# One-2-3-45/One-2-3-45

Measured on NVIDIA H100. Metric: sec/mesh end-to-end (256x256 in), lower is better.
Workload: dtype f16

## Files before the change

### one-2-3-45_b200/csrc/gemm_tc.cu

```cuda
#include <cuda.h>
#include <stdlib.h>
#include <cuda_fp16.h>

#include "common.cuh"
#include "wgmma.cuh"

namespace o2345 {
namespace {

constexpr int BM = 128, BK = 64;
constexpr int EPI_WARPS = 8;
constexpr int EPI_THREADS = 32 * EPI_WARPS;
constexpr int GEMM_THREADS = 128 + EPI_THREADS;
constexpr uint64_t WAIT_LIMIT_NS = 4000000000ull;
constexpr int MAX_CLUSTER = 8;
constexpr int RES_PREFETCH = 8;

enum { WAIT_EMPTY = 1, WAIT_FULL = 2 };

struct TrapRecord {
  unsigned long long magic;
  int tag, stage, bx, by, bz, rank, M, N, K, bn, mode, splits, conv;
};
constexpr unsigned long long TRAP_MAGIC = 0x6f32333435545250ull;
// ... 16 lines not shown
      "mbarrier.try_wait.parity.shared::cta.b64 p, [%1], %2;\n\t"
      "selp.u32 %0, 1, 0, p;\n\t}"
      : "=r"(done)
      : "r"(smem_u32(bar)), "r"(parity)
      : "memory");
  return done;
}
__device__ __forceinline__ uint64_t global_ns() {
  uint64_t t;
  asm volatile("mov.u64 %0, %%globaltimer;" : "=l"(t));
  return t;
}
__device__ __forceinline__ void tma_load_2d(void* dst, const CUtensorMap* map, uint64_t* bar, int c0, int c1) {
  asm volatile(
      "cp.async.bulk.tensor.2d.shared::cluster.global.mbarrier::complete_tx::bytes [%0], [%1, {%3, %4}], [%2];"
      ::"r"(smem_u32(dst)), "l"(map), "r"(smem_u32(bar)), "r"(c0), "r"(c1)
      : "memory");
}
__device__ __forceinline__ void tma_load_4d(void* dst, const CUtensorMap* map, uint64_t* bar, int c0, int c1, int c2, int c3) {
  asm volatile(
      "cp.async.bulk.tensor.4d.shared::cluster.global.mbarrier::complete_tx::bytes [%0], [%1, {%3, %4, %5, %6}], [%2];"
      ::"r"(smem_u32(dst)), "l"(map), "r"(smem_u32(bar)), "r"(c0), "r"(c1), "r"(c2), "r"(c3)
      : "memory");
}
__device__ __forceinline__ uint32_t cluster_ctarank() {
  uint32_t r;
  asm volatile("mov.u32 %0, %%cluster_ctarank;" : "=r"(r));
  return r;
}
__device__ __forceinline__ void cluster_sync_all() {
  asm volatile("barrier.cluster.arrive.release.aligned;\n\tbarrier.cluster.wait.acquire.aligned;" ::: "memory");
}
__device__ __forceinline__ void epi_bar() { asm volatile("bar.sync 1, 256;" ::: "memory"); }

__host__ __device__ constexpr int acc_ld(int bn) { return bn + 4; }
__device__ __forceinline__ void acc_ld32(const float* src, uint32_t (&r)[32]) {
#pragma unroll
  for (int i = 0; i < 8; ++i) {
    const float4 v = reinterpret_cast<const float4*>(src)[i];
    r[4 * i] = __float_as_uint(v.x), r[4 * i + 1] = __float_as_uint(v.y), r[4 * i + 2] = __float_as_uint(v.z), r[4 * i + 3] = __float_as_uint(v.w);
  }
}

struct GemmParams {
  int M, N, K;
  int64_t ldc;
  int nh;
  int64_t stride_c_h, stride_c_b;
  const float* bias;
  const __half* rowbias;
  int64_t rowbias_ld;
  int rows_per_group;
  const __half* residual;
  void* C;
  int out_f32;
  int act;
  float alpha;
  int batched;
  int conv, cC, cH, cW, cblocks;
  int ctaps, ctx, cox, coy, up, upa, upb;
  int splits;
  float* ws;
  int persist;
  long long* trace;
  TrapRecord* diag;
  int bn, mode;
};

__device__ __forceinline__ void stamp(const GemmParams& p, int slot) {
  if (p.trace && blockIdx.x == 0 && blockIdx.y == 0 && blockIdx.z == 0) p.trace[slot] = clock64();
}
__device__ __forceinline__ void stamp_ns(const GemmParams& p, int slot, bool any_z = false) {
  if (p.trace && blockIdx.x == 0 && blockIdx.y == 0 && (any_z || blockIdx.z == 0)) p.trace[slot] = (long long)global_ns();
}

__device__ __forceinline__ int64_t out_row(const GemmParams& p, int row) {
  if (!p.up) return row;
  const int x = row % p.cW, t = row / p.cW, y = t % p.cH, b = t / p.cH;
  return ((int64_t)b * (2 * p.cH) + 2 * y + p.upa) * (2 * p.cW) + 2 * x + p.upb;
}

__device__ __noinline__ void wait_timed_out(const GemmParams& p, int tag, int stage) {
  if (p.diag) {
    TrapRecord* d = p.diag;
    d->tag = tag, d->stage = stage, d->bx = blockIdx.x, d->by = blockIdx.y, d->bz = blockIdx.z, d->rank = (int)cluster_ctarank();
    d->M = p.M, d->N = p.N, d->K = p.K, d->bn = p.bn, d->mode = p.mode, d->splits = p.splits, d->conv = p.conv;
    __threadfence_system();
    d->magic = TRAP_MAGIC;
    __threadfence_system();
  }
  __trap();
}
__device__ __forceinline__ void mbar_wait(uint64_t* bar, uint32_t parity, const GemmParams& p, int tag, int stage) {
  if (mbar_try(bar, parity)) return;
  const uint64_t t0 = global_ns();
  uint32_t spins = 0;
  while (!mbar_try(bar, parity))
    if (((++spins) & 255u) == 0 && global_ns() - t0 > WAIT_LIMIT_NS) wait_timed_out(p, tag, stage);
}

__device__ __forceinline__ float gelu_erf(float x) { return 0.5f * x * (1.f + erff(x * 0.70710678118654752f)); }
__device__ __forceinline__ float gelu_erf_fast(float x) {
  const float z = fabsf(x) * 0.70710678118654752f;
  const float t = __fdividef(1.f, fmaf(0.3275911f, z, 1.f));
  const float poly = t * fmaf(t, fmaf(t, fmaf(t, fmaf(t, 1.061405429f, -1.453152027f), 1.421413741f), -0.284496736f), 0.254829592f);
  float e;
  asm("ex2.approx.ftz.f32 %0, %1;" : "=f"(e) : "f"(-z * z * 1.4426950408889634f));
  const float erf_abs = fmaf(-poly, e, 1.f);
  return 0.5f * x * (1.f + copysignf(erf_abs, x));
}
__device__ __forceinline__ float apply_act(float x, int act) {
  if (act == 1) return x / (1.f + __expf(-x));
  if (act == 2) return gelu_erf(x);
  if (act == 4) return x / (1.f + __expf(-1.702f * x));
  return x;
}

__device__ __forceinline__ void store8(const GemmParams& p, int64_t off, const float (&v)[8]) {
  if (p.out_f32) {
    float* o = reinterpret_cast<float*>(p.C) + off;
    *reinterpret_cast<float4*>(o) = make_float4(v[0], v[1], v[2], v[3]);
    *reinterpret_cast<float4*>(o + 4) = make_float4(v[4], v[5], v[6], v[7]);
  } else {
    __half2 h[4];
#pragma unroll
    for (int e = 0; e < 4; ++e) h[e] = __floats2half2_rn(v[2 * e], v[2 * e + 1]);
    *reinterpret_cast<uint4*>(reinterpret_cast<__half*>(p.C) + off) = *reinterpret_cast<uint4*>(h);
  }
}

__device__ __forceinline__ void epilogue_chunk(const GemmParams& p, const uint32_t (&r)[32], int row, int64_t crow, int col0) {
  const __half* rb = p.rowbias ? p.rowbias + (int64_t)(row / p.rows_per_group) * p.rowbias_ld : nullptr;
  if (p.act == 3) {
    if (col0 >= p.N) return;
    float v[16];
#pragma unroll
    for (int e = 0; e < 16; ++e) {
      float a = __uint_as_float(r[e]) * p.alpha, g = __uint_as_float(r[16 + e]) * p.alpha;
      if (p.bias) a += __ldg(p.bias + col0 + e), g += __ldg(p.bias + col0 + 16 + e);
      v[e] = a * gelu_erf(g);
    }
    const int64_t o = crow + (col0 >> 1);
    float lo[8], hi[8];
#pragma unroll
    for (int e = 0; e < 8; ++e) lo[e] = v[e], hi[e] = v[8 + e];
    store8(p, o, lo);
    store8(p, o + 8, hi);
    return;
  }
#pragma unroll
  for (int j = 0; j < 32; j += 8) {
    const int col = col0 + j;
    if (col >= p.N) break;
    float v[8];
    const bool full = col + 8 <= p.N;
    if (full && rb) {
      uint4 q = *reinterpret_cast<const uint4*>(rb + col);
      const __half* h = reinterpret_cast<const __half*>(&q);
#pragma unroll
      for (int e = 0; e < 8; ++e) v[e] = __half2float(h[e]);
    } else {
#pragma unroll
      for (int e = 0; e < 8; ++e) v[e] = (rb && col + e < p.N) ? __half2float(rb[col + e]) : 0.f;
    }
#pragma unroll
    for (int e = 0; e < 8; ++e) {
      float x = fmaf(__uint_as_float(r[j + e]), p.alpha, v[e]);
      if (p.bias && col + e < p.N) x += __ldg(p.bias + col + e);
      v[e] = apply_act(x, p.act);
    }
    if (full && (p.ldc & 7) == 0) {
      if (p.residual) {
        uint4 q = *reinterpret_cast<const uint4*>(p.residual + crow + col);
        const __half* h = reinterpret_cast<const __half*>(&q);
#pragma unroll
        for (int e = 0; e < 8; ++e) v[e] += __half2float(h[e]);
      }
      store8(p, crow + col, v);
    } else {
      for (int e = 0; e < 8 && col + e < p.N; ++e) {
        float x = v[e];
        if (p.residual) x += __half2float(p.residual[crow + col + e]);
        if (p.out_f32) reinterpret_cast<float*>(p.C)[crow + col + e] = x;
        else reinterpret_cast<__half*>(p.C)[crow + col + e] = __float2half_rn(x);
      }
    }
  }
}

__device__ __forceinline__ void splitk_partial(const GemmParams& p, const uint32_t (&r)[32], int split, int row, int col0) {
  float* w = p.ws + ((int64_t)split * p.M + row) * p.N + col0;
  if ((p.N & 3) == 0) {
#pragma unroll
    for (int e = 0; e < 32; e += 4)
      if (col0 + e < p.N)
        __stcg(reinterpret_cast<float4*>(w + e), make_float4(__uint_as_float(r[e]), __uint_as_float(r[e + 1]),
                                                              __uint_as_float(r[e + 2]), __uint_as_float(r[e + 3])));
  } else {
#pragma unroll
    for (int e = 0; e < 32; ++e)
      if (col0 + e < p.N) __stcg(w + e, __uint_as_float(r[e]));
  }
}

template <int BN>
__device__ __forceinline__ void splitk_finalize(const GemmParams& p, int m0, int n0, int z, int te) {
  const bool vec = (p.N % 8) == 0 && (p.ldc % 8) == 0 && (!p.rowbias || (p.rowbias_ld % 8) == 0);
  const int64_t plane = (int64_t)p.M * p.N;
  if (vec) {
    constexpr int PPR = BN / 8;
    constexpr int NP = BM * PPR;
    const int share = (NP + p.splits - 1) / p.splits;
    const int i1 = min(NP, (z + 1) * share);
    constexpr bool FIXED_COLS = (EPI_THREADS % PPR) == 0;
    float bcol[8];
#pragma unroll
    for (int e = 0; e < 8; ++e) bcol[e] = 0.f;
    if (FIXED_COLS && p.bias) {
      const int i0 = z * share + te, col = n0 + (i0 - (i0 / PPR) * PPR) * 8;
      if (col < p.N) {
        const float4 b0 = __ldg(reinterpret_cast<const float4*>(p.bias + col)), b1 = __ldg(reinterpret_cast<const float4*>(p.bias + col + 4));
        bcol[0] = b0.x, bcol[1] = b0.y, bcol[2] = b0.z, bcol[3] = b0.w, bcol[4] = b1.x, bcol[5] = b1.y, bcol[6] = b1.z, bcol[7] = b1.w;
      }
    }
    for (int i = z * share + te; i < i1; i += EPI_THREADS) {
      const int rl = i / PPR, row = m0 + rl, col = n0 + (i - rl * PPR) * 8;
      if (row >= p.M || col >= p.N) continue;
      const int64_t woff = (int64_t)row * p.N + col, o = out_row(p, row) * p.ldc + col;
      uint4 qb = make_uint4(0u, 0u, 0u, 0u), qr = make_uint4(0u, 0u, 0u, 0u);
      if (p.rowbias) qb = *reinterpret_cast<const uint4*>(p.rowbias + (int64_t)(row / p.rows_per_group) * p.rowbias_ld + col);
      if (p.residual) qr = *reinterpret_cast<const uint4*>(p.residual + o);
      if (!FIXED_COLS && p.bias) {
        const float4 b0 = __ldg(reinterpret_cast<const float4*>(p.bias + col)), b1 = __ldg(reinterpret_cast<const float4*>(p.bias + col + 4));
        bcol[0] = b0.x, bcol[1] = b0.y, bcol[2] = b0.z, bcol[3] = b0.w, bcol[4] = b1.x, bcol[5] = b1.y, bcol[6] = b1.z, bcol[7] = b1.w;
// ... 23 lines not shown
        v[e] = apply_act(x, p.act);
      }
      if (p.residual) {
        const __half* h = reinterpret_cast<const __half*>(&qr);
#pragma unroll
        for (int e = 0; e < 8; ++e) v[e] += __half2float(h[e]);
      }
      store8(p, o, v);
    }
    return;
  }
  const int share = (BM * BN + p.splits - 1) / p.splits;
  const int i1 = min(BM * BN, (z + 1) * share);
  for (int i = z * share + te; i < i1; i += EPI_THREADS) {
    const int rl = i / BN, row = m0 + rl, col = n0 + (i - rl * BN);
    if (row >= p.M || col >= p.N) continue;
    float x = 0.f;
    for (int s = 0; s < p.splits; ++s) x += __ldcg(p.ws + (int64_t)s * plane + (int64_t)row * p.N + col);
    x *= p.alpha;
    if (p.rowbias) x += __half2float(p.rowbias[(int64_t)(row / p.rows_per_group) * p.rowbias_ld + col]);
    if (p.bias) x += __ldg(p.bias + col);
    x = apply_act(x, p.act);
    const int64_t o = out_row(p, row) * p.ldc + col;
    if (p.residual) x += __half2float(p.residual[o]);
    if (p.out_f32) reinterpret_cast<float*>(p.C)[o] = x;
    else reinterpret_cast<__half*>(p.C)[o] = __float2half_rn(x);
  }
}

constexpr int EPI_RB_GROUPS = 8;
__host__ __device__ constexpr int epi_smem_bytes(int bn) { return bn * 4 + EPI_RB_GROUPS * bn * 2; }
__host__ __device__ constexpr int col_split(int bn) { return ((bn / 2 + 31) / 32) * 32; }

template <int BN>
__device__ __forceinline__ void epilogue_preload(const GemmParams& p, int m0, int n0, float* sbias, __half* srb, int te) {
  for (int i = te; i < BN; i += EPI_THREADS) sbias[i] = (p.bias && n0 + i < p.N) ? __ldg(p.bias + n0 + i) : 0.f;
  if (p.rowbias) {
    const int g0 = m0 / p.rows_per_group;
    const int last = (m0 + BM - 1 < p.M ? m0 + BM - 1 : p.M - 1) / p.rows_per_group;
    const int ng = last - g0 + 1;
    if (ng >= 1 && ng <= EPI_RB_GROUPS)
      for (int i = te; i < ng * BN; i += EPI_THREADS) {
        const int gi = i / BN, c = i - gi * BN;
        srb[i] = (n0 + c < p.N) ? p.rowbias[(int64_t)(g0 + gi) * p.rowbias_ld + n0 + c] : __float2half(0.f);
      }
  }
  epi_bar();
}

template <int ACT>
__device__ __forceinline__ float act_fn(float x) {
  if (ACT == 1) return __fdividef(x, 1.f + __expf(-x));
  if (ACT == 2) return gelu_erf(x);
  if (ACT == 4) return __fdividef(x, 1.f + __expf(-1.702f * x));
  return x;
}

template <int ACT>
__device__ __forceinline__ void stage_rows(const GemmParams& p, const float* acc_row, uint8_t* mine, int n0, int c_lo, int c_hi,
                                           const float* sbias, const __half* rb, bool rb_smem) {
#pragma unroll 1
  for (int c0 = c_lo; c0 < c_hi; c0 += 32) {
    if (n0 + c0 >= p.N) break;
    uint32_t r[32];
    acc_ld32(acc_row + c0, r);
    if (ACT == 3) {
      __half2 h[8];
#pragma unroll
      for (int e = 0; e < 16; e += 2) {
        float a0 = fmaf(__uint_as_float(r[e]), p.alpha, sbias[c0 + e]), a1 = fmaf(__uint_as_float(r[e + 1]), p.alpha, sbias[c0 + e + 1]);
        float g0 = fmaf(__uint_as_float(r[16 + e]), p.alpha, sbias[c0 + 16 + e]);
        float g1 = fmaf(__uint_as_float(r[17 + e]), p.alpha, sbias[c0 + 17 + e]);
        h[e >> 1] = __floats2half2_rn(a0 * gelu_erf_fast(g0), a1 * gelu_erf_fast(g1));
      }
      uint4* d = reinterpret_cast<uint4*>(mine + (c0 - c_lo));
      d[0] = reinterpret_cast<uint4*>(h)[0], d[1] = reinterpret_cast<uint4*>(h)[1];
    } else {
#pragma unroll
      for (int j = 0; j < 32; j += 8) {
        float v[8];
        const float4 b0 = *reinterpret_cast<const float4*>(sbias + c0 + j), b1 = *reinterpret_cast<const float4*>(sbias + c0 + j + 4);
        v[0] = b0.x, v[1] = b0.y, v[2] = b0.z, v[3] = b0.w, v[4] = b1.x, v[5] = b1.y, v[6] = b1.z, v[7] = b1.w;
        if (rb && (rb_smem || n0 + c0 + j + 8 <= p.N)) {
          uint4 q = *reinterpret_cast<const uint4*>(rb + c0 + j);
          const __half* hq = reinterpret_cast<const __half*>(&q);
#pragma unroll
          for (int e = 0; e < 8; ++e) v[e] += __half2float(hq[e]);
        }
        __half2 h[4];
#pragma unroll
        for (int e = 0; e < 8; e += 2) {
          float x0 = fmaf(__uint_as_float(r[j + e]), p.alpha, v[e]), x1 = fmaf(__uint_as_float(r[j + e + 1]), p.alpha, v[e + 1]);
          h[e >> 1] = __floats2half2_rn(act_fn<ACT>(x0), act_fn<ACT>(x1));
        }
        *reinterpret_cast<uint4*>(mine + (c0 - c_lo + j) * 2) = *reinterpret_cast<uint4*>(h);
      }
    }
  }
}

struct WarpOut {
  int outc, stride, ppr, total, ocol0, nout;
};
template <int MODE>
__device__ __forceinline__ WarpOut warp_out(const GemmParams& p, int n0, int c_lo, int c_hi) {
  constexpr bool geglu = MODE == 1;
  WarpOut g;
  g.outc = geglu ? (c_hi - c_lo) >> 1 : (c_hi - c_lo);
  g.stride = g.outc * 2 + 16;
  g.ppr = g.outc >> 3;
  g.total = 32 * g.ppr;
  g.ocol0 = geglu ? (n0 + c_lo) >> 1 : n0 + c_lo;
  g.nout = geglu ? p.N >> 1 : p.N;
  return g;
}

__device__ __forceinline__ void prefetch_residual(const GemmParams& p, const WarpOut& g, int lane, int row0,
                                                  uint4 (&resq)[RES_PREFETCH]) {
#pragma unroll
  for (int u = 0; u < RES_PREFETCH; ++u) {
    resq[u] = make_uint4(0u, 0u, 0u, 0u);
    const int pp = lane + 32 * u;
    if (p.residual && pp < g.total) {
      const int rl = pp / g.ppr, ci = pp - rl * g.ppr;
      const int grow = row0 + rl, col = g.ocol0 + ci * 8;
      if (grow < p.M && col < g.nout) resq[u] = *reinterpret_cast<const uint4*>(p.residual + out_row(p, grow) * p.ldc + col);
    }
  }
}

__device__ __forceinline__ uint4 add_h8(uint4 v, uint4 q) {
  __half2* a = reinterpret_cast<__half2*>(&v);
  const __half2* b = reinterpret_cast<const __half2*>(&q);
#pragma unroll
  for (int e = 0; e < 4; ++e) {
    float2 fa = __half22float2(a[e]), fb = __half22float2(b[e]);
    a[e] = __floats2half2_rn(fa.x + fb.x, fa.y + fb.y);
  }
  return v;
}

template <int BN, int MODE>
__device__ __forceinline__ void epilogue_staged(const GemmParams& p, const WarpOut& g, const float* acc_row, uint8_t* slab, int lane,
                                                int m0, int row0, int n0, int c_lo, int c_hi, const float* sbias, const __half* srb,
                                                const uint4 (&resq)[RES_PREFETCH]) {
  const int row = row0 + lane;
  const __half* rb = nullptr;
  bool rb_smem = false;
  if (MODE != 1 && p.rowbias) {
    const int rr = row < p.M ? row : p.M - 1;
    const int g0 = m0 / p.rows_per_group, last = (m0 + BM - 1 < p.M ? m0 + BM - 1 : p.M - 1) / p.rows_per_group;
    rb_smem = last - g0 + 1 <= EPI_RB_GROUPS;
    rb = rb_smem ? srb + (rr / p.rows_per_group - g0) * BN : p.rowbias + (int64_t)(rr / p.rows_per_group) * p.rowbias_ld + n0;
  }
  uint8_t* mine = slab + lane * g.stride;
  if (MODE == 0) {
    stage_rows<0>(p, acc_row, mine, n0, c_lo, c_hi, sbias, rb, rb_smem);
  } else if (MODE == 1) {
    stage_rows<3>(p, acc_row, mine, n0, c_lo, c_hi, sbias, rb, rb_smem);
  } else {
    switch (p.act) {
      case 1: stage_rows<1>(p, acc_row, mine, n0, c_lo, c_hi, sbias, rb, rb_smem); break;
      case 2: stage_rows<2>(p, acc_row, mine, n0, c_lo, c_hi, sbias, rb, rb_smem); break;
      default: stage_rows<4>(p, acc_row, mine, n0, c_lo, c_hi, sbias, rb, rb_smem); break;
    }
  }
  __syncwarp();
  __half* C = reinterpret_cast<__half*>(p.C);
#pragma unroll
  for (int u = 0; u < RES_PREFETCH; ++u) {
    const int pp = lane + 32 * u;
    if (pp < g.total) {
      const int rl = pp / g.ppr, ci = pp - rl * g.ppr;
      const int grow = row0 + rl, col = g.ocol0 + ci * 8;
      if (grow < p.M && col < g.nout) {
        uint4 v = *reinterpret_cast<const uint4*>(slab + rl * g.stride + ci * 16);
        if (p.residual) v = add_h8(v, resq[u]);
        *reinterpret_cast<uint4*>(C + out_row(p, grow) * p.ldc + col) = v;
      }
    }
  }
  constexpr int UN = 4;
  for (int base = lane + 32 * RES_PREFETCH; base < g.total; base += 32 * UN) {
    uint4 v[UN], q[UN];
    int64_t o[UN];
    bool ok[UN];
#pragma unroll
    for (int u = 0; u < UN; ++u) {
      const int pp = base + 32 * u;
      const int rl = pp / g.ppr, ci = pp - rl * g.ppr;
      const int grow = row0 + rl, col = g.ocol0 + ci * 8;
      ok[u] = pp < g.total && grow < p.M && col < g.nout;
      o[u] = out_row(p, grow) * p.ldc + col;
      if (ok[u]) {
        v[u] = *reinterpret_cast<const uint4*>(slab + rl * g.stride + ci * 16);
        if (p.residual) q[u] = *reinterpret_cast<const uint4*>(p.residual + o[u]);
      }
    }
#pragma unroll
    for (int u = 0; u < UN; ++u) {
      if (!ok[u]) continue;
      if (p.residual) v[u] = add_h8(v[u], q[u]);
      *reinterpret_cast<uint4*>(C + o[u]) = v[u];
    }
  }
}

__host__ __device__ constexpr int epi_slab_bytes(int bn) { return EPI_WARPS * 32 * (col_split(bn) * 2 + 16); }
constexpr int smem_bytes(int bn, int stages) {
  return stages * (BM * BK * 2 + bn * BK * 2) + epi_slab_bytes(bn) + 2 * stages * 8 + 16 + epi_smem_bytes(bn) + 1024;
}

struct ProducerPos {
  int x, y, b;
  int tap, tx, ty;
  int cb;
};
__device__ __forceinline__ ProducerPos producer_start(const GemmParams& p, int m0, int bz, int kb0) {
  ProducerPos q;
  q.x = q.y = q.b = q.tap = q.tx = q.ty = q.cb = 0;
  if (p.conv) {
    const int r = m0 / p.cW;
    q.x = m0 - r * p.cW, q.y = r % p.cH, q.b = r / p.cH;
    q.tap = kb0 / p.cblocks, q.cb = kb0 - q.tap * p.cblocks;
    q.ty = q.tap / p.ctx, q.tx = q.tap - q.ty * p.ctx;
  } else if (p.batched) {
    q.y = bz % p.nh, q.b = bz / p.nh;
  }
  return q;
}
__device__ __forceinline__ void producer_step(const GemmParams& p, ProducerPos& q) {
  if (p.conv && ++q.cb == p.cblocks) {
    q.cb = 0, ++q.tap;
    if (++q.tx == p.ctx) q.tx = 0, ++q.ty;
  }
}

template <int BN>
__device__ __forceinline__ void produce_stage(const GemmParams& p, const CUtensorMap* tmA, const CUtensorMap* tmB, uint8_t* a_dst,
                                              uint8_t* b_dst, uint64_t* full_bar, int kb, int m0, int n0, const ProducerPos& q) {
  mbar_expect_tx(full_bar, BM * BK * 2 + BN * BK * 2);
  if (p.conv) {
    const int c0 = q.cb * BK;
    tma_load_4d(a_dst, tmA, full_bar, c0, q.x + q.tx + p.cox, q.y + q.ty + p.coy, q.b);
    tma_load_2d(b_dst, tmB, full_bar, q.tap * p.cC + c0, n0);
  } else if (p.batched) {
    tma_load_4d(a_dst, tmA, full_bar, kb * BK, m0, q.y, q.b);
    tma_load_4d(b_dst, tmB, full_bar, kb * BK, n0, q.y, q.b);
  } else {
    tma_load_2d(a_dst, tmA, full_bar, kb * BK, m0);
    tma_load_2d(b_dst, tmB, full_bar, kb * BK, n0);
  }
}

template <int BN>
__device__ __forceinline__ void acc_store(float* acc, const float (&d)[BN / 2], int row0, int t) {
  const int r = row0 + 16 * (t >> 5) + ((t & 31) >> 2), c = 2 * (t & 3);
#pragma unroll
  for (int j = 0; j < BN / 8; ++j) {
    *reinterpret_cast<float2*>(acc + r * acc_ld(BN) + 8 * j + c) = make_float2(d[4 * j], d[4 * j + 1]);
    *reinterpret_cast<float2*>(acc + (r + 8) * acc_ld(BN) + 8 * j + c) = make_float2(d[4 * j + 2], d[4 * j + 3]);
  }
}

template <int BN, int STAGES, int MODE>
__global__ void __launch_bounds__(GEMM_THREADS, 1)
gemm_tc_kernel(const __grid_constant__ CUtensorMap tmA, const __grid_constant__ CUtensorMap tmB, const __grid_constant__ GemmParams p) {
  extern __shared__ __align__(1024) uint8_t smem_raw[];
  uint8_t* smem = reinterpret_cast<uint8_t*>((reinterpret_cast<uintptr_t>(smem_raw) + 1023) & ~(uintptr_t)1023);
  constexpr int A_BYTES = BM * BK * 2, B_BYTES = BN * BK * 2;
  static_assert(B_BYTES % 1024 == 0, "stage bases must stay 1024-byte aligned for SWIZZLE_128B");
  static_assert(BN % 32 == 0 && BN >= 64 && BN <= 256, "tile width: a multiple of 32 (GEGLU chunks, 32-column epilogue reads)");
  static_assert(BM * acc_ld(BN) * 4 <= STAGES * (A_BYTES + B_BYTES), "the accumulator tile must fit in the operand ring");
  constexpr int CSPLIT = col_split(BN);
  uint8_t* sA = smem;
  uint8_t* sB = smem + STAGES * A_BYTES;
  uint8_t* slabs = sB + STAGES * B_BYTES;
  uint64_t* full = reinterpret_cast<uint64_t*>(slabs + epi_slab_bytes(BN));
  uint64_t* empty = full + STAGES;
  float* sbias = reinterpret_cast<float*>((reinterpret_cast<uintptr_t>(empty + STAGES) + 15) & ~(uintptr_t)15);
  __half* srb = reinterpret_cast<__half*>(sbias + BN);
  float* acc = reinterpret_cast<float*>(smem);

  const int warp = threadIdx.x >> 5, lane = threadIdx.x & 31;
  if (threadIdx.x == 0) stamp(p, 0), stamp_ns(p, 16);
  const int bz = blockIdx.z;
  const int nk = p.conv ? p.ctaps * p.cblocks : (p.K + BK - 1) / BK;
  const bool split = MODE == 3 && p.splits > 1;
  int kb0 = 0, kb1 = nk;
  if (split) {
    kb0 = (int)((int64_t)nk * bz / p.splits);
    kb1 = (int)((int64_t)nk * (bz + 1) / p.splits);
  }

  if (threadIdx.x == 0) {
    asm volatile("prefetch.tensormap [%0];" ::"l"(&tmA) : "memory");
    asm volatile("prefetch.tensormap [%0];" ::"l"(&tmB) : "memory");
    for (int s = 0; s < STAGES; ++s) mbar_init(full + s, 1), mbar_init(empty + s, 2);
    asm volatile("fence.mbarrier_init.release.cluster;" ::: "memory");
    asm volatile("fence.proxy.async.shared::cta;" ::: "memory");
  }
  __syncthreads();
  pdl_wait();
  pdl_trigger();
  if (threadIdx.x == 0) stamp(p, 1);

  const int tiles_m = (p.M + BM - 1) / BM, tiles = tiles_m * ((p.N + BN - 1) / BN);
  const bool persist = MODE != 3 && p.persist;
  uint32_t cnt = 0;
  for (int t = persist ? blockIdx.x : blockIdx.y * tiles_m + blockIdx.x; t < tiles; t += persist ? gridDim.x : tiles) {
  const int m0 = (t % tiles_m) * BM, n0 = (t / tiles_m) * BN;
  if (warp < 4) {
    if (threadIdx.x == 0) {
      asm volatile("fence.proxy.async.shared::cta;" ::: "memory");
      ProducerPos q = producer_start(p, m0, bz, kb0);
      for (int kb = kb0; kb < kb1; ++kb) {
        const uint32_t c = cnt + (kb - kb0);
        const int s = c % STAGES;
        const uint32_t ph = (c / STAGES) & 1;
        mbar_wait(empty + s, ph ^ 1, p, WAIT_EMPTY, s);
        produce_stage<BN>(p, &tmA, &tmB, sA + s * A_BYTES, sB + s * B_BYTES, full + s, kb, m0, n0, q);
        producer_step(p, q);
        if (kb == kb0) stamp(p, 2);
      }
      stamp(p, 3);
    }
    __syncwarp();
  } else {
    const int wg = (warp >> 2) - 1, e = warp - 4, quarter = e & 3, te = threadIdx.x - 128;
    const int c_lo = e < 4 ? 0 : CSPLIT, c_hi = e < 4 ? CSPLIT : BN;
    const int row0 = m0 + quarter * 32;
    if (MODE != 3) epilogue_preload<BN>(p, m0, n0, sbias, srb, te);
    {
      float d[BN / 2];
#pragma unroll
      for (int i = 0; i < BN / 2; ++i) d[i] = 0.f;
      for (int kb = kb0; kb < kb1; ++kb) {
        const uint32_t c = cnt + (kb - kb0);
        const int s = c % STAGES;
        const uint32_t ph = (c / STAGES) & 1;
        mbar_wait(full + s, ph, p, WAIT_FULL, s);
        if (kb == kb0 && te == 0) stamp(p, 4);
        const uint32_t a0 = smem_u32(sA + s * A_BYTES) + wg * (64 * 128), b0 = smem_u32(sB + s * B_BYTES);
        wg::fence();
#pragma unroll
        for (int k = 0; k < BK / 16; ++k)
          wg::mma_f16<BN>(d, wg::desc_sw128(a0 + k * 32), wg::desc_sw128(b0 + k * 32), 1);
        wg::commit();
        wg::wait<1>();
        if (kb > kb0 && (threadIdx.x & 127) == 0) mbar_arrive(empty + (c - 1) % STAGES);
      }
      wg::wait<0>();
      if ((threadIdx.x & 127) == 0) mbar_arrive(empty + (cnt + kb1 - kb0 - 1) % STAGES);
      if (te == 0) stamp(p, 5);
      epi_bar();
      acc_store<BN>(acc, d, 64 * wg, threadIdx.x & 127);
    }
    epi_bar();
    if (te == 0) stamp(p, 6);
    const float* acc_row = acc + (quarter * 32 + lane) * acc_ld(BN);
    if (MODE != 3) {
      const WarpOut g = warp_out<MODE>(p, n0, c_lo, c_hi);
      uint4 resq[RES_PREFETCH];
      prefetch_residual(p, g, lane, row0, resq);
      epilogue_staged<BN, MODE>(p, g, acc_row, slabs + e * 32 * (CSPLIT * 2 + 16), lane, m0, row0, n0, c_lo, c_hi, sbias, srb, resq);
    } else {
      const int row = row0 + lane;
      if (split) {
        if (te == 0) stamp_ns(p, 17);
#pragma unroll 1
        for (int c0 = c_lo; c0 < c_hi; c0 += 32) {
          uint32_t r[32];
          acc_ld32(acc_row + c0, r);
          if (row < p.M) splitk_partial(p, r, bz, row, n0 + c0);
        }
        if (te == 0) stamp_ns(p, 18);
      } else {
        const int64_t crow = (p.batched ? (int64_t)(bz % p.nh) * p.stride_c_h + (int64_t)(bz / p.nh) * p.stride_c_b : 0) +
                             out_row(p, row < p.M ? row : 0) * p.ldc;
#pragma unroll 1
        for (int c0 = c_lo; c0 < c_hi; c0 += 32) {
          uint32_t r[32];
          acc_ld32(acc_row + c0, r);
          if (row < p.M) epilogue_chunk(p, r, row, crow, n0 + c0);
        }
      }
    }
    if (te == 0) stamp(p, 7);
  }
  cnt += kb1 - kb0;
  __syncthreads();
  }
  if (split) {
    cluster_sync_all();
    if (warp >= 4) {
      if (threadIdx.x == 128) stamp_ns(p, 21, true);
      splitk_finalize<BN>(p, blockIdx.x * BM, blockIdx.y * BN, bz, threadIdx.x - 128);
      if (threadIdx.x == 128) stamp_ns(p, 22, true);
    }
  }
  if (threadIdx.x == 0) stamp(p, 8);
}

typedef CUresult (*EncodeTiledFn)(CUtensorMap*, CUtensorMapDataType, cuuint32_t, void*, const cuuint64_t*, const cuuint64_t*,
                                  const cuuint32_t*, const cuuint32_t*, CUtensorMapInterleave, CUtensorMapSwizzle,
                                  CUtensorMapL2promotion, CUtensorMapFloatOOBfill);

EncodeTiledFn encode_fn() {
  static EncodeTiledFn fn = nullptr;
  if (!fn) {
    void* p = nullptr;
    cudaDriverEntryPointQueryResult q;
    if (cudaGetDriverEntryPoint("cuTensorMapEncodeTiled", &p, cudaEnableDefault, &q) == cudaSuccess && q == cudaDriverEntryPointSuccess)
      fn = reinterpret_cast<EncodeTiledFn>(p);
  }
  return fn;
}

int make_map(CUtensorMap* m, const void* ptr, int64_t rows, int64_t K, int64_t ld, int nh, int nb, int64_t sh, int64_t sb,
             int box_rows) {
  EncodeTiledFn fn = encode_fn();
  if (!fn) { set_error("cuTensorMapEncodeTiled entry point not available"); return O2345_ECUDA; }
  cuuint64_t dims[4] = {(cuuint64_t)K, (cuuint64_t)rows, (cuuint64_t)(nh > 0 ? nh : 1), (cuuint64_t)(nb > 0 ? nb : 1)};
  cuuint64_t strides[3] = {(cuuint64_t)ld * 2, (cuuint64_t)sh * 2, (cuuint64_t)sb * 2};
// ... 67 lines not shown

Config pick_config(const GemmParams& p, int nk, bool can_split, int64_t ws_floats) {
  read_force_env();
  Config c;
  const int M = p.M, N = p.N;
  c.persist = 0;
  if (p.batched) {
    c.bn = N <= 64 ? 64 : 128, c.splits = 1;
    return c;
  }
  static const int kBn[4] = {64, 128, 160, 256};
  static const int kSplits[6] = {1, 2, 3, 4, 6, 8};
  const bool split_ok = can_split && p.act != 3 && p.ws && 2 * (int64_t)M * N <= ws_floats;
  const int max_planes = split_ok ? (int)(ws_floats / ((int64_t)M * N)) : 1;
  float best = 1e30f;
  c.bn = 128, c.splits = 1;
  for (int bi = 0; bi < 4; ++bi) {
    const int bn = kBn[bi];
    if (bn > 64 && N <= 64) continue;
    if (g_force[1] > 0 && bn != g_force[1]) continue;
    for (int si = 0; si < 6; ++si) {
      const int sp = kSplits[si];
      if (g_force[2] > 0 && sp != (g_force[2] > nk ? nk : g_force[2])) continue;
      if (sp > 1 && (!split_ok || sp > max_planes || sp > MAX_CLUSTER || nk / sp < 3)) continue;
      const float us = predict_us(M, N, nk, bn, sp);
      if (us < best) best = us, c.bn = bn, c.splits = sp;
    }
  }
  if (best > 1e29f) {
    c.bn = (g_force[1] == 64 || g_force[1] == 128 || g_force[1] == 160 || g_force[1] == 256) ? g_force[1] : 128;
    c.splits = 1;
  }
  const int tiles = cdiv(M, BM) * cdiv(N, c.bn);
  const int min_tiles = g_persist_min_tiles > 0 ? g_persist_min_tiles : 4 * sm_count();
  c.persist = c.splits == 1 && (g_persist == 1 || (g_persist == 0 && tiles >= min_tiles));
  return c;
}

int pick_mode(const GemmParams& p, const Config& c) {
  const int nout = p.act == 3 ? p.N / 2 : p.N;
  const bool staged = !p.out_f32 && c.splits <= 1 && !p.batched && (nout % 8) == 0 && (p.ldc % 8) == 0 && ((uintptr_t)p.C % 16) == 0 &&
                      (!p.residual || ((uintptr_t)p.residual % 16) == 0);
  if (!staged) return 3;
  return p.act == 0 ? 0 : (p.act == 3 ? 1 : 2);
}

long long* g_trace = nullptr;

template <int BN, int STAGES, int MODE>
int launch(const CUtensorMap& a, const CUtensorMap& b, GemmParams p, int batch, int persist, cudaStream_t st) {
  constexpr int SMEM = smem_bytes(BN, STAGES);
  static_assert(SMEM <= 227 * 1024, "one CTA per SM");
  static PerDeviceOnce attr;
  if (attr.need())
    O2345_CUDA(cudaFuncSetAttribute(gemm_tc_kernel<BN, STAGES, MODE>, cudaFuncAttributeMaxDynamicSharedMemorySize, SMEM));
  p.bn = BN, p.mode = MODE;
  p.diag = diag_buffer(st);
  const int splits = (MODE == 3 && batch == 0 && p.splits > 1) ? p.splits : 1;
  p.splits = splits;
  dim3 grid(cdiv(p.M, BM), cdiv(p.N, BN), batch > 0 ? batch : splits);
  p.persist = MODE != 3 && batch == 0 && splits == 1 && persist;
  if (p.persist) {
    const int tiles = (int)grid.x * (int)grid.y;
    grid = dim3(tiles < sm_count() ? tiles : sm_count(), 1, 1);
  }
  O2345_CUDA(launch_pdl_cluster(gemm_tc_kernel<BN, STAGES, MODE>, grid, dim3(GEMM_THREADS), (size_t)SMEM, st, 1, splits, a, b, p));
  O2345_LAUNCH_CHECK();
// ... 172 lines not shown
```

Baseline: 2.436.

## Stage epilogue straight from registers and drop per-tile CTA barrier in persistent GEMM

The epilogue now writes the WGMMA accumulator fragments directly into the per-warp output slabs, so the full fp32 tile no longer round-trips through the operand ring. Because the ring is not reused for the accumulator, the per-tile __syncthreads and the producer's proxy fence are removed, which lets the TMA producer run ahead into the next tile while the epilogue drains. Bias and row-bias preloads move to cp.async with zero-fill, residual rows are prefetched into L2 during the first k-block, and the persistent threshold drops from four waves to just over one wave. The risks are heavier register pressure from keeping fragments live through the epilogue, scattered half2 shared-memory writes, and ordering hazards between the epilogue and the producer refilling stages.

```diff
diff --git a/one-2-3-45_b200/csrc/gemm_tc.cu b/one-2-3-45_b200/csrc/gemm_tc.cu
--- a/one-2-3-45_b200/csrc/gemm_tc.cu
+++ b/one-2-3-45_b200/csrc/gemm_tc.cu
@@ -72,15 +72,6 @@
   asm volatile("barrier.cluster.arrive.release.aligned;\n\tbarrier.cluster.wait.acquire.aligned;" ::: "memory");
 }
 __device__ __forceinline__ void epi_bar() { asm volatile("bar.sync 1, 256;" ::: "memory"); }
-
-__host__ __device__ constexpr int acc_ld(int bn) { return bn + 4; }
-__device__ __forceinline__ void acc_ld32(const float* src, uint32_t (&r)[32]) {
-#pragma unroll
-  for (int i = 0; i < 8; ++i) {
-    const float4 v = reinterpret_cast<const float4*>(src)[i];
-    r[4 * i] = __float_as_uint(v.x), r[4 * i + 1] = __float_as_uint(v.y), r[4 * i + 2] = __float_as_uint(v.z), r[4 * i + 3] = __float_as_uint(v.w);
-  }
-}
 
 struct GemmParams {
   int M, N, K;
@@ -110,6 +101,9 @@
 __device__ __forceinline__ void stamp(const GemmParams& p, int slot) {
   if (p.trace && blockIdx.x == 0 && blockIdx.y == 0 && blockIdx.z == 0) p.trace[slot] = clock64();
 }
+__device__ __forceinline__ void stamp_tile(const GemmParams& p, int it, int k) {
+  if (p.trace && it < 2 && blockIdx.x == 0 && blockIdx.y == 0 && blockIdx.z == 0) p.trace[24 + 4 * it + k] = clock64();
+}
 __device__ __forceinline__ void stamp_ns(const GemmParams& p, int slot, bool any_z = false) {
   if (p.trace && blockIdx.x == 0 && blockIdx.y == 0 && (any_z || blockIdx.z == 0)) p.trace[slot] = (long long)global_ns();
 }
@@ -169,77 +163,61 @@
   }
 }
 
-__device__ __forceinline__ void epilogue_chunk(const GemmParams& p, const uint32_t (&r)[32], int row, int64_t crow, int col0) {
-  const __half* rb = p.rowbias ? p.rowbias + (int64_t)(row / p.rows_per_group) * p.rowbias_ld : nullptr;
-  if (p.act == 3) {
-    if (col0 >= p.N) return;
-    float v[16];
-#pragma unroll
-    for (int e = 0; e < 16; ++e) {
-      float a = __uint_as_float(r[e]) * p.alpha, g = __uint_as_float(r[16 + e]) * p.alpha;
-      if (p.bias) a += __ldg(p.bias + col0 + e), g += __ldg(p.bias + col0 + 16 + e);
-      v[e] = a * gelu_erf(g);
-    }
-    const int64_t o = crow + (col0 >> 1);
-    float lo[8], hi[8];
-#pragma unroll
-    for (int e = 0; e < 8; ++e) lo[e] = v[e], hi[e] = v[8 + e];
-    store8(p, o, lo);
-    store8(p, o + 8, hi);
-    return;
-  }
-#pragma unroll
-  for (int j = 0; j < 32; j += 8) {
-    const int col = col0 + j;
-    if (col >= p.N) break;
-    float v[8];
-    const bool full = col + 8 <= p.N;
-    if (full && rb) {
-      uint4 q = *reinterpret_cast<const uint4*>(rb + col);
-      const __half* h = reinterpret_cast<const __half*>(&q);
-#pragma unroll
-      for (int e = 0; e < 8; ++e) v[e] = __half2float(h[e]);
-    } else {
-#pragma unroll
-      for (int e = 0; e < 8; ++e) v[e] = (rb && col + e < p.N) ? __half2float(rb[col + e]) : 0.f;
-    }
-#pragma unroll
-    for (int e = 0; e < 8; ++e) {
-      float x = fmaf(__uint_as_float(r[j + e]), p.alpha, v[e]);
-      if (p.bias && col + e < p.N) x += __ldg(p.bias + col + e);
-      v[e] = apply_act(x, p.act);
-    }
-    if (full && (p.ldc & 7) == 0) {
-      if (p.residual) {
-        uint4 q = *reinterpret_cast<const uint4*>(p.residual + crow + col);
-        const __half* h = reinterpret_cast<const __half*>(&q);
-#pragma unroll
-        for (int e = 0; e < 8; ++e) v[e] += __half2float(h[e]);
-      }
-      store8(p, crow + col, v);
-    } else {
-      for (int e = 0; e < 8 && col + e < p.N; ++e) {
-        float x = v[e];
-        if (p.residual) x += __half2float(p.residual[crow + col + e]);
-        if (p.out_f32) reinterpret_cast<float*>(p.C)[crow + col + e] = x;
-        else reinterpret_cast<__half*>(p.C)[crow + col + e] = __float2half_rn(x);
-      }
-    }
-  }
-}
-
-__device__ __forceinline__ void splitk_partial(const GemmParams& p, const uint32_t (&r)[32], int split, int row, int col0) {
-  float* w = p.ws + ((int64_t)split * p.M + row) * p.N + col0;
-  if ((p.N & 3) == 0) {
-#pragma unroll
-    for (int e = 0; e < 32; e += 4)
-      if (col0 + e < p.N)
-        __stcg(reinterpret_cast<float4*>(w + e), make_float4(__uint_as_float(r[e]), __uint_as_float(r[e + 1]),
-                                                              __uint_as_float(r[e + 2]), __uint_as_float(r[e + 3])));
-  } else {
-#pragma unroll
-    for (int e = 0; e < 32; ++e)
-      if (col0 + e < p.N) __stcg(w + e, __uint_as_float(r[e]));
+
+template <int BN>
+__device__ __forceinline__ void epilogue_generic(const GemmParams& p, const float (&d)[BN / 2], int m0, int n0, int r, int q, int bz) {
+  const int64_t cbase = p.batched ? (int64_t)(bz % p.nh) * p.stride_c_h + (int64_t)(bz / p.nh) * p.stride_c_b : 0;
+#pragma unroll
+  for (int h = 0; h < 2; ++h) {
+    const int row = m0 + r + 8 * h;
+    if (row >= p.M) continue;
+    const int64_t crow = cbase + out_row(p, row) * p.ldc;
+    const __half* rb = p.rowbias ? p.rowbias + (int64_t)(row / p.rows_per_group) * p.rowbias_ld : nullptr;
+#pragma unroll
+    for (int j = 0; j < BN / 8; ++j) {
+#pragma unroll
+      for (int e = 0; e < 2; ++e) {
+        const int col = n0 + 8 * j + 2 * q + e;
+        if (col >= p.N) continue;
+        float x;
+        int64_t o;
+        if (p.act == 3) {
+          if ((j & 3) >= 2) continue;
+          float a = d[4 * j + 2 * h + e] * p.alpha, g = d[4 * (j + 2) + 2 * h + e] * p.alpha;
+          if (p.bias) a += __ldg(p.bias + col), g += __ldg(p.bias + col + 16);
+          x = a * gelu_erf(g);
+          o = crow + ((n0 + 32 * (j >> 2)) >> 1) + 8 * (j & 3) + 2 * q + e;
+        } else {
+          x = fmaf(d[4 * j + 2 * h + e], p.alpha, rb ? __half2float(rb[col]) : 0.f);
+          if (p.bias) x += __ldg(p.bias + col);
+          x = apply_act(x, p.act);
+          o = crow + col;
+          if (p.residual) x += __half2float(p.residual[o]);
+        }
+        if (p.out_f32) reinterpret_cast<float*>(p.C)[o] = x;
+        else reinterpret_cast<__half*>(p.C)[o] = __float2half_rn(x);
+      }
+    }
+  }
+}
+
+template <int BN>
+__device__ __forceinline__ void splitk_partial(const GemmParams& p, const float (&d)[BN / 2], int split, int m0, int n0, int r, int q) {
+#pragma unroll
+  for (int h = 0; h < 2; ++h) {
+    const int row = m0 + r + 8 * h;
+    if (row >= p.M) continue;
+    float* w = p.ws + ((int64_t)split * p.M + row) * p.N;
+#pragma unroll
+    for (int j = 0; j < BN / 8; ++j) {
+      const int col = n0 + 8 * j + 2 * q;
+      if ((p.N & 1) == 0) {
+        if (col < p.N) __stcg(reinterpret_cast<float2*>(w + col), make_float2(d[4 * j + 2 * h], d[4 * j + 2 * h + 1]));
+      } else {
+        if (col < p.N) __stcg(w + col, d[4 * j + 2 * h]);
+        if (col + 1 < p.N) __stcg(w + col + 1, d[4 * j + 2 * h + 1]);
+      }
+    }
   }
 }
 
@@ -329,20 +307,29 @@
 __host__ __device__ constexpr int epi_smem_bytes(int bn) { return bn * 4 + EPI_RB_GROUPS * bn * 2; }
 __host__ __device__ constexpr int col_split(int bn) { return ((bn / 2 + 31) / 32) * 32; }
 
+template <int BYTES>
+__device__ __forceinline__ void cp_async_zfill(void* dst, const void* src, bool valid) {
+  asm volatile("cp.async.ca.shared.global [%0], [%1], %2, %3;" ::"r"(smem_u32(dst)), "l"(src), "n"(BYTES), "r"(valid ? BYTES : 0)
+               : "memory");
+}
+
 template <int BN>
 __device__ __forceinline__ void epilogue_preload(const GemmParams& p, int m0, int n0, float* sbias, __half* srb, int te) {
-  for (int i = te; i < BN; i += EPI_THREADS) sbias[i] = (p.bias && n0 + i < p.N) ? __ldg(p.bias + n0 + i) : 0.f;
+  for (int i = te; i < BN; i += EPI_THREADS) {
+    if (p.bias) cp_async_zfill<4>(sbias + i, p.bias + (n0 + i < p.N ? n0 + i : 0), n0 + i < p.N);
+    else sbias[i] = 0.f;
+  }
   if (p.rowbias) {
     const int g0 = m0 / p.rows_per_group;
     const int last = (m0 + BM - 1 < p.M ? m0 + BM - 1 : p.M - 1) / p.rows_per_group;
     const int ng = last - g0 + 1;
     if (ng >= 1 && ng <= EPI_RB_GROUPS)
-      for (int i = te; i < ng * BN; i += EPI_THREADS) {
-        const int gi = i / BN, c = i - gi * BN;
-        srb[i] = (n0 + c < p.N) ? p.rowbias[(int64_t)(g0 + gi) * p.rowbias_ld + n0 + c] : __float2half(0.f);
-      }
-  }
-  epi_bar();
+      for (int i = te; i < ng * (BN / 8); i += EPI_THREADS) {
+        const int gi = i / (BN / 8), c = (i - gi * (BN / 8)) * 8;
+        const bool in = n0 + c < p.N;
+        cp_async_zfill<16>(srb + gi * BN + c, p.rowbias + (int64_t)(g0 + gi) * p.rowbias_ld + (in ? n0 + c : 0), in);
+      }
+  }
 }
 
 template <int ACT>
@@ -351,49 +338,6 @@
   if (ACT == 2) return gelu_erf(x);
   if (ACT == 4) return __fdividef(x, 1.f + __expf(-1.702f * x));
   return x;
-}
-
-template <int ACT>
-__device__ __forceinline__ void stage_rows(const GemmParams& p, const float* acc_row, uint8_t* mine, int n0, int c_lo, int c_hi,
-                                           const float* sbias, const __half* rb, bool rb_smem) {
-#pragma unroll 1
-  for (int c0 = c_lo; c0 < c_hi; c0 += 32) {
-    if (n0 + c0 >= p.N) break;
-    uint32_t r[32];
-    acc_ld32(acc_row + c0, r);
-    if (ACT == 3) {
-      __half2 h[8];
-#pragma unroll
-      for (int e = 0; e < 16; e += 2) {
-        float a0 = fmaf(__uint_as_float(r[e]), p.alpha, sbias[c0 + e]), a1 = fmaf(__uint_as_float(r[e + 1]), p.alpha, sbias[c0 + e + 1]);
-        float g0 = fmaf(__uint_as_float(r[16 + e]), p.alpha, sbias[c0 + 16 + e]);
-        float g1 = fmaf(__uint_as_float(r[17 + e]), p.alpha, sbias[c0 + 17 + e]);
-        h[e >> 1] = __floats2half2_rn(a0 * gelu_erf_fast(g0), a1 * gelu_erf_fast(g1));
-      }
-      uint4* d = reinterpret_cast<uint4*>(mine + (c0 - c_lo));
-      d[0] = reinterpret_cast<uint4*>(h)[0], d[1] = reinterpret_cast<uint4*>(h)[1];
-    } else {
-#pragma unroll
-      for (int j = 0; j < 32; j += 8) {
-        float v[8];
-        const float4 b0 = *reinterpret_cast<const float4*>(sbias + c0 + j), b1 = *reinterpret_cast<const float4*>(sbias + c0 + j + 4);
-        v[0] = b0.x, v[1] = b0.y, v[2] = b0.z, v[3] = b0.w, v[4] = b1.x, v[5] = b1.y, v[6] = b1.z, v[7] = b1.w;
-        if (rb && (rb_smem || n0 + c0 + j + 8 <= p.N)) {
-          uint4 q = *reinterpret_cast<const uint4*>(rb + c0 + j);
-          const __half* hq = reinterpret_cast<const __half*>(&q);
-#pragma unroll
-          for (int e = 0; e < 8; ++e) v[e] += __half2float(hq[e]);
-        }
-        __half2 h[4];
-#pragma unroll
-        for (int e = 0; e < 8; e += 2) {
-          float x0 = fmaf(__uint_as_float(r[j + e]), p.alpha, v[e]), x1 = fmaf(__uint_as_float(r[j + e + 1]), p.alpha, v[e + 1]);
-          h[e >> 1] = __floats2half2_rn(act_fn<ACT>(x0), act_fn<ACT>(x1));
-        }
-        *reinterpret_cast<uint4*>(mine + (c0 - c_lo + j) * 2) = *reinterpret_cast<uint4*>(h);
-      }
-    }
-  }
 }
 
 struct WarpOut {
@@ -426,6 +370,13 @@
   }
 }
 
+__device__ __forceinline__ void residual_to_l2(const GemmParams& p, const WarpOut& g, int lane, int row0) {
+  const int row = row0 + lane, n = min(g.outc, g.nout - g.ocol0);
+  if (!p.residual || row >= p.M || n <= 0) return;
+  asm volatile("cp.async.bulk.prefetch.L2.global [%0], %1;" ::"l"(p.residual + out_row(p, row) * p.ldc + g.ocol0), "r"(n * 2)
+               : "memory");
+}
+
 __device__ __forceinline__ uint4 add_h8(uint4 v, uint4 q) {
   __half2* a = reinterpret_cast<__half2*>(&v);
   const __half2* b = reinterpret_cast<const __half2*>(&q);
@@ -437,32 +388,78 @@
   return v;
 }
 
-template <int BN, int MODE>
-__device__ __forceinline__ void epilogue_staged(const GemmParams& p, const WarpOut& g, const float* acc_row, uint8_t* slab, int lane,
-                                                int m0, int row0, int n0, int c_lo, int c_hi, const float* sbias, const __half* srb,
-                                                const uint4 (&resq)[RES_PREFETCH]) {
-  const int row = row0 + lane;
-  const __half* rb = nullptr;
+__host__ __device__ constexpr int epi_slab_bytes(int bn) { return EPI_WARPS * 32 * (col_split(bn) * 2 + 16); }
+
+template <int BN, int ACT>
+__device__ __forceinline__ void stage_fragment(const GemmParams& p, const float (&d)[BN / 2], uint8_t* slabs, int m0, int n0, int r,
+                                               int q, const float* sbias, const __half* srb) {
+  constexpr int CSPLIT = col_split(BN);
+  const __half* rb[2] = {nullptr, nullptr};
   bool rb_smem = false;
-  if (MODE != 1 && p.rowbias) {
-    const int rr = row < p.M ? row : p.M - 1;
+  if (ACT != 3 && p.rowbias) {
     const int g0 = m0 / p.rows_per_group, last = (m0 + BM - 1 < p.M ? m0 + BM - 1 : p.M - 1) / p.rows_per_group;
     rb_smem = last - g0 + 1 <= EPI_RB_GROUPS;
-    rb = rb_smem ? srb + (rr / p.rows_per_group - g0) * BN : p.rowbias + (int64_t)(rr / p.rows_per_group) * p.rowbias_ld + n0;
-  }
-  uint8_t* mine = slab + lane * g.stride;
+#pragma unroll
+    for (int h = 0; h < 2; ++h) {
+      const int row = m0 + r + 8 * h, rr = row < p.M ? row : p.M - 1;
+      rb[h] = rb_smem ? srb + (rr / p.rows_per_group - g0) * BN : p.rowbias + (int64_t)(rr / p.rows_per_group) * p.rowbias_ld + n0;
+    }
+  }
+  uint8_t* slab_lo = slabs + (r >> 5) * 32 * (CSPLIT * 2 + 16);
+  const int rs = r & 31;
+#pragma unroll
+  for (int j = 0; j < BN / 8; ++j) {
+    const int c = 8 * j + 2 * q;
+    constexpr bool geglu = ACT == 3;
+    const bool hi = 8 * j >= CSPLIT;
+    const int c_lo = hi ? CSPLIT : 0;
+    const int outc = geglu ? (hi ? BN - CSPLIT : CSPLIT) / 2 : (hi ? BN - CSPLIT : CSPLIT);
+    const int stride = outc * 2 + 16;
+    uint8_t* slab = slab_lo + (hi ? 4 * 32 * (CSPLIT * 2 + 16) : 0);
+    if (geglu) {
+      if ((j & 3) >= 2) continue;
+      const int oc = ((8 * (j & ~3) - c_lo) >> 1) + 8 * (j & 3) + 2 * q;
+      const float2 bv = *reinterpret_cast<const float2*>(sbias + c), bg = *reinterpret_cast<const float2*>(sbias + c + 16);
+#pragma unroll
+      for (int h = 0; h < 2; ++h) {
+        const float a0 = fmaf(d[4 * j + 2 * h], p.alpha, bv.x), a1 = fmaf(d[4 * j + 2 * h + 1], p.alpha, bv.y);
+        const float g0 = fmaf(d[4 * (j + 2) + 2 * h], p.alpha, bg.x), g1 = fmaf(d[4 * (j + 2) + 2 * h + 1], p.alpha, bg.y);
+        *reinterpret_cast<__half2*>(slab + (rs + 8 * h) * stride + oc * 2) = __floats2half2_rn(a0 * gelu_erf_fast(g0), a1 * gelu_erf_fast(g1));
+      }
+    } else {
+      const float2 bv = *reinterpret_cast<const float2*>(sbias + c);
+#pragma unroll
+      for (int h = 0; h < 2; ++h) {
+        float v0 = bv.x, v1 = bv.y;
+        if (rb[h] && (rb_smem || n0 + 8 * j + 8 <= p.N)) {
+          const float2 f = __half22float2(*reinterpret_cast<const __half2*>(rb[h] + c));
+          v0 += f.x, v1 += f.y;
+        }
+        const float x0 = fmaf(d[4 * j + 2 * h], p.alpha, v0), x1 = fmaf(d[4 * j + 2 * h + 1], p.alpha, v1);
+        *reinterpret_cast<__half2*>(slab + (rs + 8 * h) * stride + (c - c_lo) * 2) = __floats2half2_rn(act_fn<ACT>(x0), act_fn<ACT>(x1));
+      }
+    }
+  }
+}
+
+template <int BN, int MODE>
+__device__ __forceinline__ void epilogue_front(const GemmParams& p, const float (&d)[BN / 2], uint8_t* slabs, int m0, int n0, int r,
+                                               int q, const float* sbias, const __half* srb) {
   if (MODE == 0) {
-    stage_rows<0>(p, acc_row, mine, n0, c_lo, c_hi, sbias, rb, rb_smem);
+    stage_fragment<BN, 0>(p, d, slabs, m0, n0, r, q, sbias, srb);
   } else if (MODE == 1) {
-    stage_rows<3>(p, acc_row, mine, n0, c_lo, c_hi, sbias, rb, rb_smem);
+    stage_fragment<BN, 3>(p, d, slabs, m0, n0, r, q, sbias, srb);
   } else {
     switch (p.act) {
-      case 1: stage_rows<1>(p, acc_row, mine, n0, c_lo, c_hi, sbias, rb, rb_smem); break;
-      case 2: stage_rows<2>(p, acc_row, mine, n0, c_lo, c_hi, sbias, rb, rb_smem); break;
-      default: stage_rows<4>(p, acc_row, mine, n0, c_lo, c_hi, sbias, rb, rb_smem); break;
-    }
-  }
-  __syncwarp();
+      case 1: stage_fragment<BN, 1>(p, d, slabs, m0, n0, r, q, sbias, srb); break;
+      case 2: stage_fragment<BN, 2>(p, d, slabs, m0, n0, r, q, sbias, srb); break;
+      default: stage_fragment<BN, 4>(p, d, slabs, m0, n0, r, q, sbias, srb); break;
+    }
+  }
+}
+
+__device__ __forceinline__ void store_slab(const GemmParams& p, const WarpOut& g, const uint8_t* slab, int lane, int row0,
+                                           const uint4 (&resq)[RES_PREFETCH]) {
   __half* C = reinterpret_cast<__half*>(p.C);
 #pragma unroll
   for (int u = 0; u < RES_PREFETCH; ++u) {
@@ -503,7 +500,6 @@
   }
 }
 
-__host__ __device__ constexpr int epi_slab_bytes(int bn) { return EPI_WARPS * 32 * (col_split(bn) * 2 + 16); }
 constexpr int smem_bytes(int bn, int stages) {
   return stages * (BM * BK * 2 + bn * BK * 2) + epi_slab_bytes(bn) + 2 * stages * 8 + 16 + epi_smem_bytes(bn) + 1024;
 }
@@ -550,16 +546,6 @@
   }
 }
 
-template <int BN>
-__device__ __forceinline__ void acc_store(float* acc, const float (&d)[BN / 2], int row0, int t) {
-  const int r = row0 + 16 * (t >> 5) + ((t & 31) >> 2), c = 2 * (t & 3);
-#pragma unroll
-  for (int j = 0; j < BN / 8; ++j) {
-    *reinterpret_cast<float2*>(acc + r * acc_ld(BN) + 8 * j + c) = make_float2(d[4 * j], d[4 * j + 1]);
-    *reinterpret_cast<float2*>(acc + (r + 8) * acc_ld(BN) + 8 * j + c) = make_float2(d[4 * j + 2], d[4 * j + 3]);
-  }
-}
-
 template <int BN, int STAGES, int MODE>
 __global__ void __launch_bounds__(GEMM_THREADS, 1)
 gemm_tc_kernel(const __grid_constant__ CUtensorMap tmA, const __grid_constant__ CUtensorMap tmB, const __grid_constant__ GemmParams p) {
@@ -568,7 +554,6 @@
   constexpr int A_BYTES = BM * BK * 2, B_BYTES = BN * BK * 2;
   static_assert(B_BYTES % 1024 == 0, "stage bases must stay 1024-byte aligned for SWIZZLE_128B");
   static_assert(BN % 32 == 0 && BN >= 64 && BN <= 256, "tile width: a multiple of 32 (GEGLU chunks, 32-column epilogue reads)");
-  static_assert(BM * acc_ld(BN) * 4 <= STAGES * (A_BYTES + B_BYTES), "the accumulator tile must fit in the operand ring");
   constexpr int CSPLIT = col_split(BN);
   uint8_t* sA = smem;
   uint8_t* sB = smem + STAGES * A_BYTES;
@@ -577,7 +562,6 @@
   uint64_t* empty = full + STAGES;
   float* sbias = reinterpret_cast<float*>((reinterpret_cast<uintptr_t>(empty + STAGES) + 15) & ~(uintptr_t)15);
   __half* srb = reinterpret_cast<__half*>(sbias + BN);
-  float* acc = reinterpret_cast<float*>(smem);
 
   const int warp = threadIdx.x >> 5, lane = threadIdx.x & 31;
   if (threadIdx.x == 0) stamp(p, 0), stamp_ns(p, 16);
@@ -605,11 +589,11 @@
   const int tiles_m = (p.M + BM - 1) / BM, tiles = tiles_m * ((p.N + BN - 1) / BN);
   const bool persist = MODE != 3 && p.persist;
   uint32_t cnt = 0;
+  int it = 0;
   for (int t = persist ? blockIdx.x : blockIdx.y * tiles_m + blockIdx.x; t < tiles; t += persist ? gridDim.x : tiles) {
   const int m0 = (t % tiles_m) * BM, n0 = (t / tiles_m) * BN;
   if (warp < 4) {
     if (threadIdx.x == 0) {
-      asm volatile("fence.proxy.async.shared::cta;" ::: "memory");
       ProducerPos q = producer_start(p, m0, bz, kb0);
       for (int kb = kb0; kb < kb1; ++kb) {
         const uint32_t c = cnt + (kb - kb0);
@@ -618,75 +602,62 @@
         mbar_wait(empty + s, ph ^ 1, p, WAIT_EMPTY, s);
         produce_stage<BN>(p, &tmA, &tmB, sA + s * A_BYTES, sB + s * B_BYTES, full + s, kb, m0, n0, q);
         producer_step(p, q);
-        if (kb == kb0) stamp(p, 2);
+        if (kb == kb0) stamp(p, 2), stamp_tile(p, it, 3);
       }
       stamp(p, 3);
     }
     __syncwarp();
   } else {
-    const int wg = (warp >> 2) - 1, e = warp - 4, quarter = e & 3, te = threadIdx.x - 128;
-    const int c_lo = e < 4 ? 0 : CSPLIT, c_hi = e < 4 ? CSPLIT : BN;
-    const int row0 = m0 + quarter * 32;
+    const int wg = (warp >> 2) - 1, e = warp - 4, te = threadIdx.x - 128;
+    const int r = 64 * wg + 16 * (e & 3) + (lane >> 2), q = lane & 3;
     if (MODE != 3) epilogue_preload<BN>(p, m0, n0, sbias, srb, te);
-    {
-      float d[BN / 2];
-#pragma unroll
-      for (int i = 0; i < BN / 2; ++i) d[i] = 0.f;
-      for (int kb = kb0; kb < kb1; ++kb) {
-        const uint32_t c = cnt + (kb - kb0);
-        const int s = c % STAGES;
-        const uint32_t ph = (c / STAGES) & 1;
-        mbar_wait(full + s, ph, p, WAIT_FULL, s);
-        if (kb == kb0 && te == 0) stamp(p, 4);
-        const uint32_t a0 = smem_u32(sA + s * A_BYTES) + wg * (64 * 128), b0 = smem_u32(sB + s * B_BYTES);
-        wg::fence();
-#pragma unroll
-        for (int k = 0; k < BK / 16; ++k)
-          wg::mma_f16<BN>(d, wg::desc_sw128(a0 + k * 32), wg::desc_sw128(b0 + k * 32), 1);
-        wg::commit();
-        wg::wait<1>();
-        if (kb > kb0 && (threadIdx.x & 127) == 0) mbar_arrive(empty + (c - 1) % STAGES);
-      }
-      wg::wait<0>();
-      if ((threadIdx.x & 127) == 0) mbar_arrive(empty + (cnt + kb1 - kb0 - 1) % STAGES);
-      if (te == 0) stamp(p, 5);
+    float d[BN / 2];
+#pragma unroll
+    for (int i = 0; i < BN / 2; ++i) d[i] = 0.f;
+    for (int kb = kb0; kb < kb1; ++kb) {
+      const uint32_t c = cnt + (kb - kb0);
+      const int s = c % STAGES;
+      const uint32_t ph = (c / STAGES) & 1;
+      mbar_wait(full + s, ph, p, WAIT_FULL, s);
+      if (kb == kb0 && te == 0) stamp(p, 4), stamp_tile(p, it, 0);
+      const uint32_t a0 = smem_u32(sA + s * A_BYTES) + wg * (64 * 128), b0 = smem_u32(sB + s * B_BYTES);
+      wg::fence();
+#pragma unroll
+      for (int k = 0; k < BK / 16; ++k)
+        wg::mma_f16<BN>(d, wg::desc_sw128(a0 + k * 32), wg::desc_sw128(b0 + k * 32), 1);
+      wg::commit();
+      wg::wait<1>();
+      if (kb > kb0 && (threadIdx.x & 127) == 0) mbar_arrive(empty + (c - 1) % STAGES);
+      if (MODE != 3 && kb == kb0) {
+        residual_to_l2(p, warp_out<MODE>(p, n0, e < 4 ? 0 : CSPLIT, e < 4 ? CSPLIT : BN), lane, m0 + (e & 3) * 32);
+      }
+    }
+    wg::wait<0>();
+    if ((threadIdx.x & 127) == 0) mbar_arrive(empty + (cnt + kb1 - kb0 - 1) % STAGES);
+    if (te == 0) stamp(p, 5), stamp_tile(p, it, 1);
+    if (MODE != 3) {
+      const int c_lo = e < 4 ? 0 : CSPLIT, c_hi = e < 4 ? CSPLIT : BN;
+      const int row0 = m0 + (e & 3) * 32;
+      const WarpOut g = warp_out<MODE>(p, n0, c_lo, c_hi);
+      asm volatile("cp.async.wait_all;" ::: "memory");
       epi_bar();
-      acc_store<BN>(acc, d, 64 * wg, threadIdx.x & 127);
-    }
-    epi_bar();
-    if (te == 0) stamp(p, 6);
-    const float* acc_row = acc + (quarter * 32 + lane) * acc_ld(BN);
-    if (MODE != 3) {
-      const WarpOut g = warp_out<MODE>(p, n0, c_lo, c_hi);
+      if (te == 0) stamp(p, 6);
+      epilogue_front<BN, MODE>(p, d, slabs, m0, n0, r, q, sbias, srb);
       uint4 resq[RES_PREFETCH];
       prefetch_residual(p, g, lane, row0, resq);
-      epilogue_staged<BN, MODE>(p, g, acc_row, slabs + e * 32 * (CSPLIT * 2 + 16), lane, m0, row0, n0, c_lo, c_hi, sbias, srb, resq);
+      epi_bar();
+      store_slab(p, g, slabs + e * 32 * (CSPLIT * 2 + 16), lane, row0, resq);
+    } else if (split) {
+      if (te == 0) stamp_ns(p, 17);
+      splitk_partial<BN>(p, d, bz, m0, n0, r, q);
+      if (te == 0) stamp_ns(p, 18);
     } else {
-      const int row = row0 + lane;
-      if (split) {
-        if (te == 0) stamp_ns(p, 17);
-#pragma unroll 1
-        for (int c0 = c_lo; c0 < c_hi; c0 += 32) {
-          uint32_t r[32];
-          acc_ld32(acc_row + c0, r);
-          if (row < p.M) splitk_partial(p, r, bz, row, n0 + c0);
-        }
-        if (te == 0) stamp_ns(p, 18);
-      } else {
-        const int64_t crow = (p.batched ? (int64_t)(bz % p.nh) * p.stride_c_h + (int64_t)(bz / p.nh) * p.stride_c_b : 0) +
-                             out_row(p, row < p.M ? row : 0) * p.ldc;
-#pragma unroll 1
-        for (int c0 = c_lo; c0 < c_hi; c0 += 32) {
-          uint32_t r[32];
-          acc_ld32(acc_row + c0, r);
-          if (row < p.M) epilogue_chunk(p, r, row, crow, n0 + c0);
-        }
-      }
-    }
-    if (te == 0) stamp(p, 7);
+      epilogue_generic<BN>(p, d, m0, n0, r, q, bz);
+    }
+    if (te == 0) stamp(p, 7), stamp_tile(p, it, 2);
   }
   cnt += kb1 - kb0;
-  __syncthreads();
+  ++it;
   }
   if (split) {
     cluster_sync_all();
@@ -820,7 +791,7 @@
     c.splits = 1;
   }
   const int tiles = cdiv(M, BM) * cdiv(N, c.bn);
-  const int min_tiles = g_persist_min_tiles > 0 ? g_persist_min_tiles : 4 * sm_count();
+  const int min_tiles = g_persist_min_tiles > 0 ? g_persist_min_tiles : sm_count() + 1;
   c.persist = c.splits == 1 && (g_persist == 1 || (g_persist == 0 && tiles >= min_tiles));
   return c;
 }
```

Result: no change. 2.433, median of 6 (-0.1%).
